# EntityOfCode/eoc-tfhe

Hardware: AMD Instinct MI355X
Metric: gate bootstraps/sec (HomNAND) (higher is better)
Workload: dtype f64

## Files before the change

eoc_tfhe_amd/csrc/blind_rotate_pair.inc:

```
    extern __shared__ __attribute__((aligned(16))) unsigned char smem[];
    d2 *s_tw = reinterpret_cast<d2 *>(smem);
    d2 *s_twist = s_tw + kTwEntries;
    d2 *s_scr_all = s_twist + kNH;

    const int tid = threadIdx.x, lane = tid & 63;
    const int h = __builtin_amdgcn_readfirstlane(tid >> 6);
    d2 *scr = s_scr_all + h * kScr;
    d2 *scr_partner = s_scr_all + (h ^ 1) * kScr;
    int32_t *ext = reinterpret_cast<int32_t *>(scr);

    const uint32_t job = blockIdx.x;
    typedef const __attribute__((address_space(4))) uint32_t *cu32p;
    unsigned long long bara_addr = (unsigned long long)(uintptr_t)(A.bara + (size_t)job * A.bara_stride);

    load_tables(s_tw, s_twist, g_tw, g_twist, tid, 128);
    if (A.prep && A.step_begin == 0) {
        const uint32_t gjob = A.job0 + job, g = gjob / A.ks_S;
        prepare_row(A.inline_desc ? A.desc0 : A.ks_descs[g], gjob - g * A.ks_S, A.n, A.bara + (size_t)job * A.bara_stride, tid, 128);
        if constexpr (SABAR) eoc_row_stores_to_l2();
        __syncthreads();
        if constexpr (SABAR) eoc_scalar_cache_acquire();
    }
    asm volatile("" : "+s"(bara_addr));
    const cu32p bara32 = (cu32p)bara_addr;
    uint16_t *s_abar = reinterpret_cast<uint16_t *>(s_scr_all + 2 * kScr);
    if constexpr (!SABAR) {
        const uint32_t *bara_v = reinterpret_cast<const uint32_t *>(A.bara + (size_t)job * A.bara_stride);
        for (int m = tid; m < (A.n + 2) / 2; m += 128) reinterpret_cast<uint32_t *>(s_abar)[m] = bara_v[m];
        __syncthreads();
    }
    auto load_abar = [&](int idx) __attribute__((always_inline)) {
        if constexpr (SABAR) return (int)((bara32[idx >> 1] >> ((idx & 1) * 16)) & 0xffffu);
        else return (int)s_abar[idx];
    };

    uint32_t racc[16];
    {
        const int barb = load_abar(A.n);
        const int rot = (2 * kN - barb) & (2 * kN - 1);
        const int32_t *st = A.acc_state + ((size_t)job * 2 + h) * kN;
        const int32_t *tvj = TV ? tv + (size_t)((A.job0 + job) / tv_rows) * kN : nullptr;
#pragma unroll
        for (int r = 0; r < 16; r++) {
            int j = lane + 64 * (r & 7) + (r >> 3) * kNH;
            int idx = (j - rot) & (2 * kN - 1);
            int32_t v;
            if constexpr (TV) {
                const uint32_t c = (uint32_t)tvj[idx & (kN - 1)];
                v = (int32_t)((idx & kN) ? 0u - c : c);
            } else {
                v = (idx & kN) ? -A.mu : A.mu;
            }
            v = h ? v : 0;
            if (A.step_begin > 0) v = st[j];
            racc[r] = (uint32_t)v;
        }
    }
    __syncthreads();

    const int Bgbit = BGBIT > 0 ? BGBIT : A.Bgbit;
    const uint32_t Bg = 1u << Bgbit, maskBg = Bg - 1, halfBg = Bg >> 1;
    uint32_t offset = 0;
#pragma unroll
    for (int p = 1; p <= L; p++) offset += halfBg << (32 - p * Bgbit);
    constexpr int KPL = 2 * L;
    const __amdgpu_buffer_rsrc_t bk_rsrc =
        __builtin_amdgcn_make_buffer_rsrc(const_cast<double *>(A.bkfft), 0, (int)((size_t)A.n * KPL * 2 * kNH * 16), 0x00020000);
    const double bias1 = 4503599627370496.0 + (double)halfBg, bias2 = 4503599627370496.0 + (double)Bg;

#ifdef EOC_STAMPS
    unsigned long long st_acc[16] = {0, 0, 0, 0, 0, 0, 0, 0, 0, 0, 0, 0, 0, 0, 0, 0};
    unsigned long long st_prev = __builtin_amdgcn_s_memtime();
    st_acc[12] = st_prev;
    st_acc[14] = __builtin_amdgcn_s_getreg((4) | (0 << 6) | (31 << 11));
    st_acc[13] = __builtin_amdgcn_s_getreg((20) | (0 << 6) | (31 << 11));
#endif
    const int prio_slot = __builtin_amdgcn_s_getreg((4) | (0 << 6) | (3 << 11));
    constexpr bool kResT2 = L == 2;
    d2 res_t2[4];
    if constexpr (kResT2) tw_load(res_t2, s_tw + kTwF2 + lane, 64);
    constexpr bool kResT1 = L == 2;
    d2 res_t1[4];
    if constexpr (kResT1) tw_load(res_t1, s_tw + kTwI1 + (lane & 7), 8);
    int abar_next = load_abar(A.step_begin);
    for (int i = A.step_begin; i < A.step_end; i++) {
        EOC_STAMP(15);
        if (A.prio_duty >= 0) {
            const bool first_part = (i & 15) < A.prio_duty;
            if (first_part == ((prio_slot & 1) != 0))
                __builtin_amdgcn_s_setprio(1);
            else
                __builtin_amdgcn_s_setprio(0);
        } else if (A.prio_duty <= -2) {
            const unsigned long long now = __builtin_amdgcn_s_memtime();
            if ((int)((now >> (-A.prio_duty)) & 1) == (prio_slot & 1))
                __builtin_amdgcn_s_setprio(1);
            else
                __builtin_amdgcn_s_setprio(0);
        }
        const int abar = __builtin_amdgcn_readfirstlane(abar_next);
        abar_next = load_abar(i + 1);
        auto load_row = [&](int p, int c, d2 (&b)[8]) __attribute__((always_inline)) {
            const uint32_t row_off = (uint32_t)((((size_t)i * KPL + h * L) * 2 + (size_t)(p - 1) * 2 + c) * kNH * 16);
#pragma unroll
            for (int r = 0; r < 8; r++)
                b[r] = __builtin_bit_cast(d2, __builtin_amdgcn_raw_buffer_load_b128(bk_rsrc, lane * 16, (int)(row_off + r * 1024), 0));
        };
        d2 ra[8], rb[8];
        uint32_t dlo[8], dhi[8];
        {
            const int s = abar & 63;
            const int src = ((lane - s) & 63) << 2;
            uint32_t t[16], d[16];
#pragma unroll
            for (int r = 0; r < 16; r++) t[r] = (uint32_t)__builtin_amdgcn_ds_bpermute(src, (int)racc[r]);
            const bool borrow = lane < s;
#define EOC_RQ(q) case q: rot_digits<q>(t, racc, borrow, offset, d); break;
            switch (abar >> 6) {
                EOC_RQ(0) EOC_RQ(1) EOC_RQ(2) EOC_RQ(3) EOC_RQ(4) EOC_RQ(5) EOC_RQ(6) EOC_RQ(7)
                EOC_RQ(8) EOC_RQ(9) EOC_RQ(10) EOC_RQ(11) EOC_RQ(12) EOC_RQ(13) EOC_RQ(14) EOC_RQ(15)
                EOC_RQ(16) EOC_RQ(17) EOC_RQ(18) EOC_RQ(19) EOC_RQ(20) EOC_RQ(21) EOC_RQ(22) EOC_RQ(23)
                EOC_RQ(24) EOC_RQ(25) EOC_RQ(26) EOC_RQ(27) EOC_RQ(28) EOC_RQ(29) EOC_RQ(30)
                default: rot_digits<31>(t, racc, borrow, offset, d); break;
            }
#undef EOC_RQ
#pragma unroll
            for (int r = 0; r < 8; r++) {
                dlo[r] = d[r];
                dhi[r] = d[8 + r];
            }
        }
        EOC_STAMP(0);
        auto make_x0 = [&](int p, d2 (&x)[8]) __attribute__((always_inline)) {
            const int shift = 32 - p * Bgbit;
#pragma unroll
            for (int r = 0; r < 4; r++) {
                const uint32_t ua = (dlo[r] >> shift) & maskBg, ub = (dhi[r] >> shift) & maskBg;
                const uint32_t up = (dlo[r + 4] >> shift) & maskBg, uq = (dhi[r + 4] >> shift) & maskBg;
                const double a = __hiloint2double(0x43300000, (int)ua) - bias1;
                const double b = __hiloint2double(0x43300000, (int)ub) - bias1;
                const double dm = __hiloint2double(0x43300000, (int)(up - uq + Bg)) - bias2;
                const double dp = __hiloint2double(0x43300000, (int)(up + uq)) - bias2;
                fwd_stage0(x[r], x[r + 4], a, b, dm, dp);
            }
            fwd_pass0_tail(x);
        };
        auto mac = [&](bool first, const d2 (&x)[8], const d2 (&b)[8], d2 (&acc_)[8]) __attribute__((always_inline)) {
#pragma unroll
            for (int r = 0; r < 8; r++) {
                if (first) {
                    acc_[r].x = EOC_FMA(-x[r].y, b[r].y, x[r].x * b[r].x);
                    acc_[r].y = EOC_FMA(x[r].y, b[r].x, x[r].x * b[r].y);
                } else {
                    acc_[r].x = EOC_FMA(-x[r].y, b[r].y, EOC_FMA(x[r].x, b[r].x, acc_[r].x));
                    acc_[r].y = EOC_FMA(x[r].y, b[r].x, EOC_FMA(x[r].x, b[r].y, acc_[r].y));
                }
            }
        };
        d2 xs[L][8], S[8];
#pragma unroll
        for (int p0 = 0; p0 + 1 < L; p0 += 2) {
            load_row(p0 + 1, 1 - h, ra);
            load_row(p0 + 2, 1 - h, rb);
            make_x0(p0 + 1, xs[p0]);
            EOC_STAMP(1);
            fft_fwd_rest_x2(xs[p0], xs[p0 + 1], [&]() __attribute__((always_inline)) { make_x0(p0 + 2, xs[p0 + 1]); },
                            s_tw, scr, lane, kResT2 ? &res_t2 : nullptr);
            EOC_STAMP(2);
            mac(p0 == 0, xs[p0], ra, S);
            mac(false, xs[p0 + 1], rb, S);
            EOC_STAMP(3);
        }
        if constexpr ((L & 1) != 0) {
            load_row(L, 1 - h, ra);
            make_x0(L, xs[L - 1]);
            EOC_STAMP(1);
            fft_fwd_rest(xs[L - 1], s_tw, scr, lane);
            EOC_STAMP(2);
            mac(L == 1, xs[L - 1], ra, S);
            EOC_STAMP(3);
        }
        load_row(1, h, ra);
        if constexpr (L >= 2) load_row(2, h, rb);
#pragma unroll
        for (int r = 0; r < 8; r++) scr[r * 64 + lane] = S[r];
        EOC_STAMP(4);
        __syncthreads();
        EOC_STAMP(5);
#pragma unroll
        for (int r = 0; r < 8; r++) S[r] = scr_partner[r * 64 + lane];
        mac(false, xs[0], ra, S);
        if constexpr (L >= 3) load_row(3, h, ra);
        if constexpr (L >= 2) mac(false, xs[1], rb, S);
        if constexpr (L >= 4) load_row(4, h, rb);
        if constexpr (L >= 3) mac(false, xs[2], ra, S);
        if constexpr (L >= 4) mac(false, xs[3], rb, S);
        EOC_STAMP(6);
        __syncthreads();
        EOC_STAMP(7);
        d2 ut[8];
        fft_inv_wave(S, ut, s_tw, s_twist, scr, lane, kResT1 ? &res_t1 : nullptr);
        EOC_STAMP(8);
#pragma unroll
        for (int r = 0; r < 8; r++) {
            d2 y = cmulc(S[r], ut[r]);
            racc[r] += wrap_trunc(y.x);
            racc[8 + r] += wrap_trunc(y.y);
        }
        wave_lds_fence();
        EOC_STAMP(9);
    }
    if (A.step_end >= A.n) {
#pragma unroll
        for (int r = 0; r < 16; r++) {
            const int j = lane + 64 * r;
            ext[j] = (int32_t)racc[r];
            ext[j + kN] = (int32_t)(0u - racc[r]);
        }
        wave_lds_fence();
    }
#ifdef EOC_STAMPS
    st_acc[11] = __builtin_amdgcn_s_memtime();
    if (A.stamps && lane == 0)
        for (int k = 0; k < 16; k++) A.stamps[((size_t)blockIdx.x * 2 + h) * 16 + k] = st_acc[k];
#endif

    const int lane_e = (int)__builtin_amdgcn_mbcnt_hi(~0u, __builtin_amdgcn_mbcnt_lo(~0u, 0u));
    if (A.step_end < A.n) {
        int32_t *st = A.acc_state + ((size_t)job * 2 + h) * kN;
#pragma unroll
        for (int r = 0; r < 16; r++) st[lane_e + 64 * (r & 7) + (r >> 3) * kNH] = (int32_t)racc[r];
        return;
    }
    if (MANY && !A.ks_descs) {
        const uint32_t gjob = A.job0 + job, g = gjob / tv_rows, si = gjob - g * tv_rows;
        int32_t *u0 = A.u - (size_t)A.job0 * (kN + 1) + ((size_t)g * n_tables * tv_rows + si) * (kN + 1);
        const size_t slot_stride = (size_t)tv_rows * (kN + 1);
        if (h == 0) {
            for (uint32_t jt = 0; jt < n_tables; jt++) {
                int32_t *u = u0 + jt * slot_stride;
#pragma unroll
                for (int r = 0; r < 16; r++) {
                    const int j = lane_e + 64 * r;
                    u[j] = ext[(2 * kN + (int)jt - j) & (2 * kN - 1)];
                }
            }
        } else if ((uint32_t)lane_e < n_tables) {
            u0[lane_e * slot_stride + kN] = ext[lane_e];
        }
    } else if (A.ks_descs) {
        const uint32_t gjob = A.job0 + job;
        if (h == 0) {
#pragma unroll
            for (int r = 0; r < 16; r++) {
// ... 22 lines not shown
```

eoc_tfhe_amd/csrc/engine.hip:

```cpp
#include "kernels.hip.h"
#include "canon_twiddles.h"
#include "common.h"
#include "../../include/eoc_tfhe_gpu.h"

#include <algorithm>
#include <cstdio>
#include <cstdlib>
#include <cstring>
#include <mutex>
#include <new>
#include <vector>

using namespace eoc;

#define HIP_TRY(expr)                                                                       \
    do {                                                                                    \
        hipError_t _e = (expr);                                                             \
        if (_e != hipSuccess) {                                                             \
            eoc_set_error("%s failed: %s (%s:%d)", #expr, hipGetErrorString(_e), __FILE__, \
                          __LINE__);                                                        \
            return EOC_ERR_HIP;                                                             \
        }                                                                                   \
    } while (0)

struct eoc_engine {
    int device = 0;
    eoc_params p{};
    int kpl = 0;
    size_t n1p = 0;
    d2 *d_tw = nullptr, *d_twist = nullptr;
    double *d_bkfft = nullptr;
    int32_t *d_ksk = nullptr;
    bool own_keys = false;
    const double *bkfft = nullptr;
    const int32_t *ksk = nullptr;
    void *d_ksl = nullptr;
    bool ksl_ready = false;
    struct Workspace {
        uint16_t *d_bara = nullptr;
        int32_t *d_u = nullptr;
        uint32_t *d_ubar = nullptr;
        int32_t *d_acc_state = nullptr;
        size_t ws_jobs = 0;
        GateDesc *d_descs = nullptr, *h_descs = nullptr;
        size_t ws_descs = 0, desc_pos = 0;
        hipEvent_t ring_ev = nullptr;
        bool ring_ev_set = false;
        bool ring_pushed_since_mark = false;
        GateDesc *d_persist = nullptr, *h_persist = nullptr;
        size_t persist_cap = 0, persist_pos = 0;
        int32_t *d_mixed = nullptr;
        uint32_t *h_perm = nullptr;
        hipEvent_t perm_ev = nullptr;
        size_t ws_mixed = 0;
    } ws;
    unsigned long long *d_stamps = nullptr;
    int num_cus = 256;
    int prio_duty_override = INT32_MIN;
    int prio_multi = -1;
    int br_slice = 0;
    bool no_fold = false;
    bool scalar_abar = false;
    bool no_pool = false;
    int br_parts = 0;
    int br_wide = -1;
    int bara_stride = 0;
    bool ks_waves_ok = true;
    int ks_mfma = -1;
    uint64_t stats[3] = {0, 0, 0};
    uint64_t ws_grows = 0;
    uint64_t br_launches = 0;
    uint64_t br_wide_launches = 0;
    uint64_t ks_mfma_launches = 0;
    bool profiling = false;
    struct Span { hipEvent_t a, b; int kind; };
    std::vector<Span> spans;
    double kernel_ms[3] = {0, 0, 0};
    uint64_t kernel_launches[3] = {0, 0, 0};
    std::mutex mu;
};

enum { KIND_PREPARE = 0, KIND_BLIND_ROTATE = 1, KIND_KEYSWITCH = 2 };

struct SpanGuard {
    eoc_engine *e;
    hipStream_t st;
    hipEvent_t a = nullptr, b = nullptr;
    int kind;
    SpanGuard(eoc_engine *e_, hipStream_t st_, int kind_) : e(e_), st(st_), kind(kind_)
    {
        if (!e->profiling) return;
        if (hipEventCreate(&a) != hipSuccess || hipEventCreate(&b) != hipSuccess) {
            a = b = nullptr;
            return;
        }
        hipEventRecord(a, st);
    }
    ~SpanGuard()
    {
        if (!a) return;
        hipEventRecord(b, st);
        e->spans.push_back({a, b, kind});
    }
};

static int valid_params(const eoc_params *p)
{
    if (!p) return 0;
    if (p->n < 1 || p->n > 1023) return 0;
    if (p->l < 1 || p->l > 4 || p->Bgbit < 1 || p->l * p->Bgbit > 32) return 0;
    if (((int64_t)p->l << p->Bgbit) > 8192) return 0;
    if (p->ks_t < 1 || p->ks_basebit < 1 || p->ks_basebit > 4 || p->ks_t * p->ks_basebit > 31) return 0;
    return 1;
}

extern "C" size_t eoc_bkfft_bytes(const eoc_params *p) { return (size_t)p->n * 2 * p->l * 2 * kNH * 16; }
extern "C" size_t eoc_ksk_row_stride(const eoc_params *p) { return ((size_t)p->n + 1 + 255) / 256 * 256; }
extern "C" size_t eoc_ksk_dev_bytes(const eoc_params *p)
{
    return (size_t)kN * p->ks_t * (((size_t)1 << p->ks_basebit) - 1) * eoc_ksk_row_stride(p) * 4;
// ... 53 lines not shown
        put(4 * lane, kTwI0 + 2 * 64 + lane);
        put(4 * (lane + 64), kTwI0 + 3 * 64 + lane);
    }
    for (int j = 0; j < kNH; j++) {
        twist[2 * j] = EOC_E2048[j][0];
        twist[2 * j + 1] = EOC_E2048[j][1];
    }
    HIP_TRY(hipMalloc(&e->d_tw, tw.size() * 8));
    HIP_TRY(hipMalloc(&e->d_twist, twist.size() * 8));
    HIP_TRY(hipMemcpy(e->d_tw, tw.data(), tw.size() * 8, hipMemcpyHostToDevice));
    HIP_TRY(hipMemcpy(e->d_twist, twist.data(), twist.size() * 8, hipMemcpyHostToDevice));
    HIP_TRY(hipDeviceSynchronize());
    return EOC_OK;
}

extern "C" int eoc_engine_create(int device, const eoc_params *p, eoc_engine **out)
{
    if (!out || !valid_params(p)) {
        eoc_set_error("eoc_engine_create: bad arguments (need 1 <= n <= 1023, 1 <= l <= 4, l * Bgbit <= 32, l * 2^Bgbit <= 8192 "
                      "-- the FP64 external product is not exact beyond that --, ks_t * ks_basebit <= 31, ks_basebit <= 4)");
        return EOC_ERR_ARG;
    }
    int cnt = eoc_device_count();
    if (cnt <= 0 || device < 0 || device >= cnt) {
        eoc_set_error("eoc_engine_create: no usable HIP device (count=%d, asked %d); the gate path has no CPU fallback",
                      cnt, device);
        return EOC_ERR_NO_DEVICE;
    }
    HIP_TRY(hipSetDevice(device));
    eoc_engine *e = new (std::nothrow) eoc_engine();
    if (!e) return EOC_ERR_ALLOC;
    e->device = device;
    e->p = *p;
    e->kpl = 2 * p->l;
    e->n1p = eoc_ksk_row_stride(p);
    e->bara_stride = (p->n + 1 + 31) / 32 * 32;
    int rc = upload_tables(e);
    if (rc) {
        delete e;
        return rc;
    }
    {
        int cus = 0;
        if (hipDeviceGetAttribute(&cus, hipDeviceAttributeMultiprocessorCount, device) == hipSuccess && cus > 0) e->num_cus = cus;
        if (const char *s = getenv("EOC_TFHE_PRIO_DUTY")) e->prio_duty_override = atoi(s);
        if (const char *s = getenv("EOC_TFHE_PRIO_MULTI")) e->prio_multi = atoi(s);
        if (const char *s = getenv("EOC_TFHE_BR_SLICE")) e->br_slice = atoi(s);
        if (getenv("EOC_TFHE_NO_FOLD")) e->no_fold = true;
        if (getenv("EOC_TFHE_NO_POOL")) e->no_pool = true;
        if (const char *s = getenv("EOC_TFHE_SCALAR_ABAR")) e->scalar_abar = atoi(s) != 0;
        if (const char *s = getenv("EOC_TFHE_BR_PARTS")) e->br_parts = atoi(s);
        if (const char *s = getenv("EOC_TFHE_BR_WIDE")) e->br_wide = atoi(s);
        if (const char *s = getenv("EOC_TFHE_KS_MFMA")) e->ks_mfma = atoi(s) != 0;
    }
#define EOC_KS_ATTR(TT, NWV, IWV)                                                                              \
    if (hipFuncSetAttribute(reinterpret_cast<const void *>(&k_keyswitch_waves<TT, NWV, IWV>),                  \
                            hipFuncAttributeMaxDynamicSharedMemorySize, KS3Cfg<TT, NWV, IWV>::LDS_BYTES) != hipSuccess) \
        e->ks_waves_ok = false
    EOC_KS_ATTR(8, 8, 16);
    EOC_KS_ATTR(8, 8, 32);
    EOC_KS_ATTR(8, 4, 64);
    EOC_KS_ATTR(8, 8, 64);
#undef EOC_KS_ATTR
    if (!e->ks_waves_ok) (void)hipGetLastError();
    *out = e;
    return EOC_OK;
}

static void free_ws(eoc_engine::Workspace &W)
{
    hipFree(W.d_bara);
    hipFree(W.d_u);
    hipFree(W.d_ubar);
    hipFree(W.d_acc_state);
    hipFree(W.d_descs);
    hipFree(W.d_mixed);
    if (W.h_descs) hipHostFree(W.h_descs);
    if (W.h_perm) hipHostFree(W.h_perm);
    if (W.perm_ev) hipEventDestroy(W.perm_ev);
    if (W.ring_ev) hipEventDestroy(W.ring_ev);
    hipFree(W.d_persist);
    if (W.h_persist) hipHostFree(W.h_persist);
    W = eoc_engine::Workspace();
}

extern "C" void eoc_engine_destroy(eoc_engine *e)
{
    if (!e) return;
    hipSetDevice(e->device);
    hipDeviceSynchronize();
    hipFree(e->d_tw);
    hipFree(e->d_twist);
    if (e->own_keys) {
        hipFree(e->d_bkfft);
        hipFree(e->d_ksk);
    }
    hipFree(e->d_ksl);
    free_ws(e->ws);
    hipFree(e->d_stamps);
    delete e;
}

static bool stream_is_capturing(hipStream_t st)
{
    hipStreamCaptureStatus cap = hipStreamCaptureStatusNone;
    return st && hipStreamIsCapturing(st, &cap) == hipSuccess && cap == hipStreamCaptureStatusActive;
// ... 280 lines not shown
        even(0, njobs_total, br_slice > 0 ? (uint32_t)br_slice : njobs_total, force_wide);
    else if (force_wide)
        even(0, njobs_total, resident_wide, true);
    else if (!can_wide || njobs_total <= resident_pair)
        even(0, njobs_total, resident_pair, false);
    else {
        const uint32_t full = njobs_total / resident_wide * resident_wide, rem = njobs_total - full;
        if (full) even(0, full, resident_wide, true);
        if (rem) even(full, rem, rem <= resident_pair ? resident_pair : resident_wide, rem > resident_pair);
    }
    return plan;
}

static BRArgs blind_rotate_args(const eoc_engine *e, const WS &W, const BRWork &w, const BRSeg &sg, int part, int parts)
{
    BRArgs a{};
    a.bkfft = e->bkfft;
    a.bara = W.d_bara + (size_t)sg.off * e->bara_stride;
    a.u = W.d_u + (size_t)sg.off * (kN + 1);
    a.njobs = sg.njobs;
    a.n = e->p.n;
    a.Bgbit = e->p.Bgbit;
    a.bara_stride = e->bara_stride;
    a.mu = (int32_t)(1u << 29);
    a.stamps = e->d_stamps;
    a.ks_descs = w.fold != BRWork::NONE ? w.descs : nullptr;
    a.prep = w.fold == BRWork::KS_AND_PREP;
    a.inline_desc = w.inline_desc != nullptr;
    if (w.inline_desc) {
        a.desc0 = *w.inline_desc;
        a.ks_descs = reinterpret_cast<const GateDesc *>(W.d_descs);
    }
    a.ubar = W.d_ubar;
    a.ks_S = w.fold != BRWork::NONE ? w.S : 1;
    a.ks_prec_offset = 1u << (32 - (1 + e->p.ks_basebit * e->p.ks_t));
    a.job0 = sg.off;
    a.step_begin = (int)((long long)e->p.n * part / parts);
    a.step_end = (int)((long long)e->p.n * (part + 1) / parts);
    a.acc_state = W.d_acc_state;
    const uint32_t resident = (sg.wide ? 8u : 4u) * (uint32_t)e->num_cus;
    a.prio_duty = (e->prio_duty_override != INT32_MIN) ? e->prio_duty_override
                  : (sg.njobs <= resident ? kPrioDuty : e->prio_multi);
    return a;
}

template <int L, int BGBIT> static const void *br_pair_kernel(BRWork::Seed seed, bool sabar)
{
    switch (seed) {
    case BRWork::GATE: return sabar ? (const void *)&k_blind_rotate<L, BGBIT, true> : (const void *)&k_blind_rotate<L, BGBIT, false>;
    case BRWork::TV: return sabar ? (const void *)&k_blind_rotate_tv<L, BGBIT, true> : (const void *)&k_blind_rotate_tv<L, BGBIT, false>;
    default: return sabar ? (const void *)&k_lut_many<L, BGBIT, true> : (const void *)&k_lut_many<L, BGBIT, false>;
    }
}
template <int BGBIT> static const void *br_wide_kernel(BRWork::Seed seed, bool sabar)
{
    switch (seed) {
    case BRWork::GATE: return sabar ? (const void *)&k_blind_rotate_wide<BGBIT, true> : (const void *)&k_blind_rotate_wide<BGBIT, false>;
    case BRWork::TV: return sabar ? (const void *)&k_blind_rotate_wide_tv<BGBIT, true> : (const void *)&k_blind_rotate_wide_tv<BGBIT, false>;
    default: return sabar ? (const void *)&k_lut_many_wide<BGBIT, true> : (const void *)&k_lut_many_wide<BGBIT, false>;
    }
}
struct BRKernel { const void *fn; dim3 grid, block; unsigned lds; };
static BRKernel blind_rotate_kernel(bool wide, int l, int Bgbit, bool sabar, BRWork::Seed seed, uint32_t njobs)
{
    if (wide) {
        const void *fn = Bgbit == 10 ? br_wide_kernel<10>(seed, sabar) : br_wide_kernel<0>(seed, sabar);
        return {fn, dim3((njobs + kBRWideJobsPerWG - 1) / kBRWideJobsPerWG), dim3(64 * kBRWideJobsPerWG), kBRWideLds};
    }
    const void *fn = nullptr;
    if (l == 2 && Bgbit == 10) fn = br_pair_kernel<2, 10>(seed, sabar);
    else if (l == 3 && Bgbit == 7) fn = br_pair_kernel<3, 7>(seed, sabar);
    else if (l == 1) fn = br_pair_kernel<1, 0>(seed, sabar);
    else if (l == 2) fn = br_pair_kernel<2, 0>(seed, sabar);
    else if (l == 3) fn = br_pair_kernel<3, 0>(seed, sabar);
    else if (l == 4) fn = br_pair_kernel<4, 0>(seed, sabar);
    return {fn, dim3(njobs), dim3(128), kBRLds};
}

static int launch_blind_rotate(eoc_engine *e, WS &W, const BRWork &w, hipStream_t st)
{
    const bool folds = w.fold != BRWork::NONE;
    if ((w.seed != BRWork::GATE && !w.tv) || (w.seed == BRWork::MANY && (folds || w.n_tables == 0)) ||
        (folds && !w.inline_desc && (!w.descs || !w.S)) || (w.inline_desc && (w.fold != BRWork::KS_AND_PREP || !w.S))) {
        eoc_set_error("internal: blind rotation of family %d with fold %d: a table family needs its test polynomials, the "
                      "many-LUT kernel has no fold, a fold needs descriptors and their row count", (int)w.seed, (int)w.fold);
        return EOC_ERR_STATE;
    }
    SpanGuard span(e, st, KIND_BLIND_ROTATE);
    const BRPlan plan = plan_blind_rotate(w.njobs, e->num_cus, e->p.l, e->kpl, e->p.n, e->br_slice, e->br_parts, e->br_wide);
    for (const BRSeg &sg : plan.segs) {
        const BRKernel k = blind_rotate_kernel(sg.wide, e->p.l, e->p.Bgbit, e->scalar_abar, w.seed, sg.njobs);
        if (!k.fn) return EOC_ERR_ARG;
        for (int part = 0; part < plan.parts; part++) {
            BRArgs a = blind_rotate_args(e, W, w, sg, part, plan.parts);
            void *args[] = {&a, (void *)&e->d_tw, (void *)&e->d_twist, (void *)&w.tv, (void *)&w.tv_rows, (void *)&w.n_tables};
            HIP_TRY(hipLaunchKernel(k.fn, k.grid, k.block, args, k.lds, st));
            e->br_launches++;
            e->br_wide_launches += sg.wide;
        }
    }
    return EOC_OK;
}

constexpr uint32_t kKsMfmaMinS = 1;
static int launch_keyswitch(eoc_engine *e, WS &W, const GateDesc *d_descs, uint32_t ngates, uint32_t S, hipStream_t st,
                            bool init_done, const GateDesc *inline_desc)
{
    KSArgs a;
    a.inline_desc = inline_desc != nullptr;
    if (inline_desc) a.desc0 = *inline_desc;
    else a.desc0 = GateDesc{0, 0, nullptr, nullptr, nullptr, nullptr};
    a.ksk = e->ksk;
    a.u = W.d_u;
    a.ubar = W.d_ubar;
    a.n = e->p.n;
    a.n1p = (int)e->n1p;
    a.t = e->p.ks_t;
    a.basebit = e->p.ks_basebit;
    a.S = S;
    a.mu = (int32_t)(1u << 29);
    SpanGuard span(e, st, KIND_KEYSWITCH);
    if (!init_done) {
        hipLaunchKernelGGL(k_ks_init, dim3(S, ngates), dim3(256), 0, st, d_descs, a);
        HIP_TRY(hipGetLastError());
    }
    const uint32_t ntiles = (S + KS_GT - 1) / KS_GT;
    const int ncb = (int)(e->n1p / 64);
    const int bb = e->p.ks_basebit, t = e->p.ks_t;
#define EOC_KS_LAUNCH(TT, NWV, IWV)                                                                     \
    do {                                                                                                  \
        auto kfn = k_keyswitch_waves<TT, NWV, IWV>;                                                       \
        constexpr int lds = KS3Cfg<TT, NWV, IWV>::LDS_BYTES;                                              \
        constexpr int ns = KS3Cfg<TT, NWV, IWV>::NS;                                                      \
        hipLaunchKernelGGL(kfn, dim3(ntiles * (unsigned)ncb * ns, ngates), dim3(64 * NWV), lds, st, d_descs, a); \
    } while (0)
    const bool fast = bb == 2 && t == 8 && e->ks_waves_ok;
    const bool mfma = bb == 2 && t == 8 && e->ksl_ready && (e->ks_mfma == 1 || (e->ks_mfma < 0 && S >= kKsMfmaMinS));
    if (mfma) {
        ks_mfma_launch(ks_mfma_plan(S, (int)e->n1p), ngates, d_descs, a, e->d_ksl, st);
        e->ks_mfma_launches++;
    }
    else if (fast && ncb == 4) EOC_KS_LAUNCH(8, 8, 16);
    else if (fast && ncb == 8) EOC_KS_LAUNCH(8, 8, 32);
    else if (fast && ncb == 12) EOC_KS_LAUNCH(8, 4, 64);
// ... 647 lines not shown
```

eoc_tfhe_amd/csrc/kernels.hip.h:

```cpp
#pragma once
#include <hip/hip_runtime.h>
#include <stdint.h>
#include <type_traits>

namespace eoc {

typedef double d2 __attribute__((ext_vector_type(2)));

constexpr int kN = 1024;
constexpr int kNH = 512;
constexpr int kScr = 568;
constexpr int kTwF1 = 0;
constexpr int kTwF2 = 32;
constexpr int kTwI1 = 32 + 256;
constexpr int kTwI0 = 32 + 256 + 32;
constexpr int kTwEntries = 32 + 256 + 32 + 256;

#define EOC_FMA(a, b, c) __builtin_fma((a), (b), (c))

#define EOC_SQRT_HALF 0x1.6a09e667f3bcdp-1
#define EOC_E128_RE 0x1.d906bcf328d46p-1
#define EOC_E128_IM 0x1.87de2a6aea963p-2
#define EOC_E64_RE 0x1.f6297cff75cb0p-1
#define EOC_E64_IM 0x1.8f8b83c69a60bp-3
// ... 97 lines not shown
    ct_w(x[0], x[2], t[1]);
    ct_w(x[1], x[3], t[1]);
    ct_iw(x[4], x[6], t[1]);
    ct_iw(x[5], x[7], t[1]);
    ct_w(x[0], x[1], t[2]);
    ct_iw(x[2], x[3], t[2]);
    ct_w(x[4], x[5], t[3]);
    ct_iw(x[6], x[7], t[3]);
}
__device__ __forceinline__ void t01_write(const d2 (&x)[8], d2 *scr, int lane)
{
#pragma unroll
    for (int r = 0; r < 8; r++) scr[72 * r + lane] = x[r];
    wave_lds_fence();
}
__device__ __forceinline__ void t01_read(d2 (&x)[8], const d2 *scr, int lane)
{
    const int hi = lane >> 3, lo = lane & 7;
#pragma unroll
    for (int r = 0; r < 8; r++) x[r] = scr[72 * hi + 8 * r + lo];
    wave_lds_fence();
}
__device__ __forceinline__ void t12_write(const d2 (&x)[8], d2 *scr, int lane)
{
    const int hi = lane >> 3, lo = lane & 7;
#pragma unroll
    for (int r = 0; r < 8; r++) scr[f12(hi * 64 + r * 8 + lo)] = x[r];
    wave_lds_fence();
}
__device__ __forceinline__ void t12_read(d2 (&x)[8], const d2 *scr, int lane)
{
#pragma unroll
    for (int r = 0; r < 8; r++) x[r] = scr[f12(lane * 8 + r)];
    wave_lds_fence();
}

__device__ __forceinline__ void fft_fwd_rest(d2 (&x)[8], const d2 *tw, d2 *scr, int lane)
{
    d2 t1[4], t2[4];
    tw_load(t1, tw + kTwF1 + (lane >> 3), 8);
    t01_write(x, scr, lane);
    t01_read(x, scr, lane);
    fwd_pass12(x, t1);
    t12_write(x, scr, lane);
    tw_load(t2, tw + kTwF2 + lane, 64);
    t12_read(x, scr, lane);
    fwd_pass12(x, t2);
}
#define EOC_SB() __builtin_amdgcn_sched_barrier(0)
#define EOC_SGB(mask, n) __builtin_amdgcn_sched_group_barrier((mask), (n), 0)
#define EOC_M_VALU 0x002
#define EOC_M_DSR 0x100
#define EOC_M_DSW 0x200
template <class MakeB>
__device__ __forceinline__ void fft_fwd_rest_x2(d2 (&xa)[8], d2 (&xb)[8], MakeB make_b, const d2 *tw, d2 *scr, int lane,
                                                const d2 (*T2)[4] = nullptr)
{
    d2 t1[4], t2[4];
    EOC_SB();
    tw_load(t1, tw + kTwF1 + (lane >> 3), 8);
    wave_lds_fence();
    t01_write(xa, scr, lane);
    make_b();
    t01_read(xa, scr, lane);
    EOC_SGB(EOC_M_DSR, 4);
#pragma unroll
    for (int k = 0; k < 8; k++) {
        EOC_SGB(EOC_M_DSW, 1);
        EOC_SGB(EOC_M_VALU, 10);
    }
    EOC_SGB(EOC_M_VALU, 64);
    EOC_SGB(EOC_M_DSR, 8);
    EOC_SB();
    t01_write(xb, scr, lane);
    t01_read(xb, scr, lane);
    if (T2) {
#pragma unroll
        for (int k = 0; k < 4; k++) t2[k] = (*T2)[k];
    } else {
        tw_load(t2, tw + kTwF2 + lane, 64);
    }
    wave_lds_fence();
    fwd_pass12(xa, t1);
#pragma unroll
    for (int k = 0; k < 8; k++) {
        EOC_SGB(EOC_M_DSW, 1);
        EOC_SGB(EOC_M_VALU, 4);
    }
    if (T2) EOC_SGB(EOC_M_DSR, 8);
    else EOC_SGB(EOC_M_DSR, 12);
    EOC_SGB(EOC_M_VALU, 40);
    EOC_SB();
    t12_write(xa, scr, lane);
    t12_read(xa, scr, lane);
    fwd_pass12(xb, t1);
#pragma unroll
    for (int k = 0; k < 8; k++) {
        EOC_SGB(EOC_M_DSW, 1);
        EOC_SGB(EOC_M_VALU, 4);
    }
    EOC_SGB(EOC_M_DSR, 8);
    EOC_SGB(EOC_M_VALU, 40);
    EOC_SB();
    t12_write(xb, scr, lane);
    t12_read(xb, scr, lane);
    fwd_pass12(xa, t2);
#pragma unroll
    for (int k = 0; k < 8; k++) {
        EOC_SGB(EOC_M_DSW, 1);
        EOC_SGB(EOC_M_VALU, 4);
    }
    EOC_SGB(EOC_M_DSR, 8);
    EOC_SGB(EOC_M_VALU, 40);
    EOC_SB();
    fwd_pass12(xb, t2);
}

__device__ __forceinline__ void inv_pass2(d2 (&x)[8])
{
    const d2 wc = {EOC_SQRT_HALF, EOC_SQRT_HALF};
    ct_1(x[0], x[1]);
    ct_1(x[2], x[3]);
    ct_1(x[4], x[5]);
    ct_1(x[6], x[7]);
    ct_1(x[0], x[2]);
    ct_ic(x[1], x[3]);
    ct_1(x[4], x[6]);
    ct_ic(x[5], x[7]);
    ct_1(x[0], x[4]);
    ct_wc(x[1], x[5], wc);
    ct_ic(x[2], x[6]);
    ct_iwc(x[3], x[7], wc);
}
__device__ __forceinline__ void inv_pass10(d2 (&x)[8], const d2 (&t)[4])
{
    ct_wc(x[0], x[1], t[0]);
    ct_wc(x[2], x[3], t[0]);
    ct_wc(x[4], x[5], t[0]);
    ct_wc(x[6], x[7], t[0]);
    ct_wc(x[0], x[2], t[1]);
    ct_iwc(x[1], x[3], t[1]);
    ct_wc(x[4], x[6], t[1]);
    ct_iwc(x[5], x[7], t[1]);
    ct_wc(x[0], x[4], t[2]);
    ct_wc(x[1], x[5], t[3]);
    ct_iwc(x[2], x[6], t[2]);
    ct_iwc(x[3], x[7], t[3]);
}
__device__ __forceinline__ void t21_read(d2 (&x)[8], const d2 *scr, int lane)
{
    const int hi = lane >> 3, lo = lane & 7;
#pragma unroll
    for (int r = 0; r < 8; r++) x[r] = scr[f12(hi * 64 + r * 8 + lo)];
    wave_lds_fence();
}
__device__ __forceinline__ void t10_read(d2 (&x)[8], const d2 *scr, int lane)
{
#pragma unroll
    for (int r = 0; r < 8; r++) x[r] = scr[72 * r + lane];
    wave_lds_fence();
}
__device__ __forceinline__ void fft_inv_wave(d2 (&x)[8], d2 (&ut)[8], const d2 *tw, const d2 *s_twist, d2 *scr, int lane,
                                             const d2 (*T1)[4] = nullptr)
{
    d2 t1[4], t0[4];
    EOC_SB();
    if (T1) {
#pragma unroll
        for (int k = 0; k < 4; k++) t1[k] = (*T1)[k];
    } else {
        tw_load(t1, tw + kTwI1 + (lane & 7), 8);
    }
    inv_pass2(x);
    {
        constexpr int ord[8] = {0, 4, 1, 5, 2, 6, 3, 7};
#pragma unroll
        for (int q = 0; q < 8; q++) scr[f12(lane * 8 + ord[q])] = x[ord[q]];
        wave_lds_fence();
    }
    t21_read(x, scr, lane);
    EOC_SGB(EOC_M_VALU, 32);
    EOC_SGB(EOC_M_VALU, 4);  EOC_SGB(EOC_M_DSW, 2);
    EOC_SGB(EOC_M_VALU, 6);  EOC_SGB(EOC_M_DSW, 2);
    EOC_SGB(EOC_M_VALU, 4);  EOC_SGB(EOC_M_DSW, 2);
    EOC_SGB(EOC_M_VALU, 6);  EOC_SGB(EOC_M_DSW, 2);
    EOC_SGB(EOC_M_DSR, 8);
    tw_load(t0, tw + kTwI0 + lane, 64);
#pragma unroll
    for (int r = 0; r < 8; r++) ut[r] = s_twist[lane + 64 * r];
    wave_lds_fence();
    EOC_SB();
    inv_pass10(x, t1);
    {
        constexpr int ord[8] = {0, 4, 1, 5, 2, 6, 3, 7};
        const int hi = lane >> 3, lo = lane & 7;
#pragma unroll
        for (int q = 0; q < 8; q++) scr[72 * hi + 8 * ord[q] + lo] = x[ord[q]];
        wave_lds_fence();
    }
    t10_read(x, scr, lane);
    EOC_SGB(EOC_M_VALU, 48);
#pragma unroll
    for (int k = 0; k < 4; k++) {
        EOC_SGB(EOC_M_VALU, 6);
        EOC_SGB(EOC_M_DSW, 2);
    }
    EOC_SGB(EOC_M_DSR, 8);
    EOC_SB();
    inv_pass10(x, t0);
}

__device__ __forceinline__ uint32_t wrap_trunc(double v)
{
    double m = __builtin_trunc(v) + 6755399441055744.0;
    return (uint32_t)__double2loint(m);
}

__device__ __forceinline__ void load_tables(d2 *s_tw, d2 *s_twist, const d2 *g_tw, const d2 *g_twist, int tid, int nthreads)
{
    for (int i = tid; i < kTwEntries; i += nthreads) s_tw[i] = g_tw[i];
    for (int i = tid; i < kNH; i += nthreads) s_twist[i] = g_twist[i];
}

__global__ __launch_bounds__(256) void k_fft_fwd_polys(const int32_t *__restrict__ polys,
                                                        double *__restrict__ specs, size_t count,
                                                        const d2 *__restrict__ g_tw,
                                                        const d2 *__restrict__ g_twist, double scale)
{
    __shared__ d2 s_tw[kTwEntries];
    __shared__ d2 s_scr[4][kScr];
    const int tid = threadIdx.x, lane = tid & 63, w = tid >> 6;
    for (int i = tid; i < kTwEntries; i += 256) s_tw[i] = g_tw[i];
    (void)g_twist;
    __syncthreads();
    size_t poly = (size_t)blockIdx.x * 4 + w;
    if (poly >= count) return;
    const int32_t *p = polys + poly * kN;
    d2 x[8];
#pragma unroll
    for (int r = 0; r < 4; r++) {
        int j = lane + 64 * r;
        double a = (double)p[j], b = (double)p[j + kNH], pp = (double)p[j + 256], q = (double)p[j + 256 + kNH];
// ... 173 lines not shown
        st_acc[k] += _t - st_prev;                                                        \
        st_prev = _t;                                                                     \
    } while (0)
#else
#define EOC_STAMP(k) do { } while (0)
#endif

struct BRArgs {
    const double *bkfft;
    uint16_t *bara;
    int32_t *u;
    uint32_t njobs;
    int n, Bgbit, bara_stride;
    int32_t mu;
    unsigned long long *stamps;
    int prio_duty;
    const GateDesc *ks_descs;
    GateDesc desc0;
    int inline_desc;
    int prep;
    uint32_t *ubar;
    uint32_t ks_S, ks_prec_offset, job0;
    int step_begin, step_end;
    int32_t *acc_state;
};

template <int Q>
__device__ __forceinline__ void rot_digits(const uint32_t (&t)[16], const uint32_t (&racc)[16], bool borrow, uint32_t offset,
                                           uint32_t (&d)[16])
{
#pragma unroll
    for (int r = 0; r < 16; r++) {
        const int k0 = (r - Q) & 31, k1 = (r - Q - 1) & 31;
        const uint32_t a0 = t[k0 & 15], a1 = t[k1 & 15];
        const uint32_t A = offset - racc[r];
        const bool n0 = k0 >= 16, n1 = k1 >= 16;
        if (n0 == n1) {
            const uint32_t w = borrow ? a1 : a0;
            d[r] = n0 ? A - w : A + w;
        } else {
            const uint32_t d0 = n0 ? A - a0 : A + a0, d1 = n1 ? A - a1 : A + a1;
            d[r] = borrow ? d1 : d0;
        }
    }
}
constexpr int kAbarLds = 2048;
constexpr int kBRLds = (kTwEntries + kNH + 2 * kScr) * 16 + kAbarLds;


template <int L, int BGBIT = 0, bool SABAR = false>
__global__ __launch_bounds__(128, 2) void k_blind_rotate(BRArgs A, const d2 *__restrict__ g_tw,
                                                         const d2 *__restrict__ g_twist)
{
    constexpr bool TV = false, MANY = false;
    const int32_t *const tv = nullptr;
    const uint32_t tv_rows = 1, n_tables = 1;
#include "blind_rotate_pair.inc"
}
template <int L, int BGBIT = 0, bool SABAR = false>
__global__ __launch_bounds__(128, 2) void k_blind_rotate_tv(BRArgs A, const d2 *__restrict__ g_tw,
                                                            const d2 *__restrict__ g_twist, const int32_t *__restrict__ tv,
                                                            uint32_t tv_rows)
{
    constexpr bool TV = true, MANY = false;
    const uint32_t n_tables = 1;
#include "blind_rotate_pair.inc"
}
template <int L, int BGBIT = 0, bool SABAR = false>
__global__ __launch_bounds__(128, 2) void k_lut_many(BRArgs A, const d2 *__restrict__ g_tw, const d2 *__restrict__ g_twist,
                                                     const int32_t *__restrict__ tv, uint32_t tv_rows, uint32_t n_tables)
{
    constexpr bool TV = true, MANY = true;
#include "blind_rotate_pair.inc"
}

__device__ __forceinline__ void fft_inv_x2(d2 (&xa)[8], d2 (&xb)[8], d2 (&ut)[8], const d2 *tw, const d2 *s_twist, d2 *scr,
                                           int lane)
{
    d2 t1[4], t0[4];
    const int hi = lane >> 3, lo = lane & 7;
    EOC_SB();
    tw_load(t1, tw + kTwI1 + (lane & 7), 8);
    inv_pass2(xa);
    EOC_SB();
#pragma unroll
    for (int r = 0; r < 8; r++) scr[f12(lane * 8 + r)] = xa[r];
    wave_lds_fence();
    inv_pass2(xb);
    t21_read(xa, scr, lane);
#pragma unroll
    for (int k = 0; k < 8; k++) {
        EOC_SGB(EOC_M_DSW, 1);
        EOC_SGB(EOC_M_VALU, 5);
    }
    EOC_SGB(EOC_M_VALU, 16);
    EOC_SGB(EOC_M_DSR, 8);
    EOC_SB();
#pragma unroll
    for (int r = 0; r < 8; r++) scr[f12(lane * 8 + r)] = xb[r];
    wave_lds_fence();
    t21_read(xb, scr, lane);
    tw_load(t0, tw + kTwI0 + lane, 64);
    wave_lds_fence();
    inv_pass10(xa, t1);
#pragma unroll
    for (int k = 0; k < 8; k++) {
        EOC_SGB(EOC_M_DSW, 1);
        EOC_SGB(EOC_M_VALU, 4);
    }
    EOC_SGB(EOC_M_DSR, 12);
    EOC_SGB(EOC_M_VALU, 40);
    EOC_SB();
#pragma unroll
    for (int r = 0; r < 8; r++) scr[72 * hi + 8 * r + lo] = xa[r];
    wave_lds_fence();
    t10_read(xa, scr, lane);
    inv_pass10(xb, t1);
#pragma unroll
    for (int k = 0; k < 8; k++) {
        EOC_SGB(EOC_M_DSW, 1);
        EOC_SGB(EOC_M_VALU, 4);
    }
    EOC_SGB(EOC_M_DSR, 8);
    EOC_SGB(EOC_M_VALU, 40);
    EOC_SB();
// ... 442 lines not shown
```

Measured before the change: 303,200.

## Keep L=2 blind-rotate twiddles in registers and software-pipeline bootstrapping-key row loads

For L=2 the blind-rotate kernel now loads the forward and inverse twiddles and the twist factors from global memory into registers once, and skips copying the tables into LDS. It also restructures the per-step MAC into a row-granular pipeline: bootstrapping-key rows are issued a few rows ahead, starting inside the last forward-FFT pass, and are interleaved with the MACs and the partner-scratch reads. The goal is to cut LDS traffic for twiddles and hide global-load latency. The cost is much higher register pressure, which could cause spills or lower occupancy. The old LDS-table path stays available through an environment flag.

```diff
diff --git a/eoc_tfhe_amd/csrc/blind_rotate_pair.inc b/eoc_tfhe_amd/csrc/blind_rotate_pair.inc
--- a/eoc_tfhe_amd/csrc/blind_rotate_pair.inc
+++ b/eoc_tfhe_amd/csrc/blind_rotate_pair.inc
@@ -13,7 +13,8 @@
     typedef const __attribute__((address_space(4))) uint32_t *cu32p;
     unsigned long long bara_addr = (unsigned long long)(uintptr_t)(A.bara + (size_t)job * A.bara_stride);
 
-    load_tables(s_tw, s_twist, g_tw, g_twist, tid, 128);
+    constexpr bool kResAll = L == 2 && !TLDS;
+    if constexpr (!kResAll) load_tables(s_tw, s_twist, g_tw, g_twist, tid, 128);
     if (A.prep && A.step_begin == 0) {
         const uint32_t gjob = A.job0 + job, g = gjob / A.ks_S;
         prepare_row(A.inline_desc ? A.desc0 : A.ks_descs[g], gjob - g * A.ks_S, A.n, A.bara + (size_t)job * A.bara_stride, tid, 128);
@@ -78,10 +79,19 @@
     const int prio_slot = __builtin_amdgcn_s_getreg((4) | (0 << 6) | (3 << 11));
     constexpr bool kResT2 = L == 2;
     d2 res_t2[4];
-    if constexpr (kResT2) tw_load(res_t2, s_tw + kTwF2 + lane, 64);
+    if constexpr (kResAll) tw_load(res_t2, g_tw + kTwF2 + lane, 64);
+    else if constexpr (kResT2) tw_load(res_t2, s_tw + kTwF2 + lane, 64);
     constexpr bool kResT1 = L == 2;
     d2 res_t1[4];
-    if constexpr (kResT1) tw_load(res_t1, s_tw + kTwI1 + (lane & 7), 8);
+    if constexpr (kResAll) tw_load(res_t1, g_tw + kTwI1 + (lane & 7), 8);
+    else if constexpr (kResT1) tw_load(res_t1, s_tw + kTwI1 + (lane & 7), 8);
+    d2 res_f1[4], res_i0[4], ut[8];
+    if constexpr (kResAll) {
+        tw_load(res_f1, g_tw + kTwF1 + (lane >> 3), 8);
+        tw_load(res_i0, g_tw + kTwI0 + lane, 64);
+#pragma unroll
+        for (int r = 0; r < 8; r++) ut[r] = g_twist[lane + 64 * r];
+    }
     int abar_next = load_abar(A.step_begin);
     for (int i = A.step_begin; i < A.step_end; i++) {
         EOC_STAMP(15);
@@ -106,7 +116,6 @@
             for (int r = 0; r < 8; r++)
                 b[r] = __builtin_bit_cast(d2, __builtin_amdgcn_raw_buffer_load_b128(bk_rsrc, lane * 16, (int)(row_off + r * 1024), 0));
         };
-        d2 ra[8], rb[8];
         uint32_t dlo[8], dhi[8];
         {
             const int s = abar & 63;
@@ -158,48 +167,105 @@
             }
         };
         d2 xs[L][8], S[8];
-#pragma unroll
-        for (int p0 = 0; p0 + 1 < L; p0 += 2) {
-            load_row(p0 + 1, 1 - h, ra);
-            load_row(p0 + 2, 1 - h, rb);
-            make_x0(p0 + 1, xs[p0]);
+        if constexpr (kResAll) {
+            constexpr int kRowAhead = 3;
+            const uint32_t step_off = (uint32_t)((((size_t)i * KPL + h * L) * 2) * kNH * 16);
+            d2 q[16][2];
+            auto issue = [&](int b) __attribute__((always_inline)) {
+                const uint32_t off = step_off + (uint32_t)((b < 8 ? 1 - h : h) * kNH * 16 + (b & 7) * 1024);
+                q[b][0] = __builtin_bit_cast(d2, __builtin_amdgcn_raw_buffer_load_b128(bk_rsrc, lane * 16, (int)off, 0));
+                q[b][1] = __builtin_bit_cast(d2, __builtin_amdgcn_raw_buffer_load_b128(bk_rsrc, lane * 16, (int)(off + 2 * kNH * 16), 0));
+            };
+            auto mac1 = [](d2 x, d2 b, d2 a) __attribute__((always_inline)) {
+                d2 o;
+                o.x = EOC_FMA(-x.y, b.y, EOC_FMA(x.x, b.x, a.x));
+                o.y = EOC_FMA(x.y, b.x, EOC_FMA(x.x, b.y, a.y));
+                return o;
+            };
+            make_x0(1, xs[0]);
             EOC_STAMP(1);
-            fft_fwd_rest_x2(xs[p0], xs[p0 + 1], [&]() __attribute__((always_inline)) { make_x0(p0 + 2, xs[p0 + 1]); },
-                            s_tw, scr, lane, kResT2 ? &res_t2 : nullptr);
+            fft_fwd_rest_x2(xs[0], xs[1], [&]() __attribute__((always_inline)) { make_x0(2, xs[1]); }, s_tw, scr, lane, &res_t2,
+                            &res_f1, [&]() __attribute__((always_inline)) {
+#pragma unroll
+                                for (int b = 0; b < kRowAhead; b++) issue(b);
+                            });
             EOC_STAMP(2);
-            mac(p0 == 0, xs[p0], ra, S);
-            mac(false, xs[p0 + 1], rb, S);
-            EOC_STAMP(3);
-        }
-        if constexpr ((L & 1) != 0) {
-            load_row(L, 1 - h, ra);
-            make_x0(L, xs[L - 1]);
-            EOC_STAMP(1);
-            fft_fwd_rest(xs[L - 1], s_tw, scr, lane);
-            EOC_STAMP(2);
-            mac(L == 1, xs[L - 1], ra, S);
-            EOC_STAMP(3);
-        }
-        load_row(1, h, ra);
-        if constexpr (L >= 2) load_row(2, h, rb);
-#pragma unroll
-        for (int r = 0; r < 8; r++) scr[r * 64 + lane] = S[r];
-        EOC_STAMP(4);
-        __syncthreads();
-        EOC_STAMP(5);
-#pragma unroll
-        for (int r = 0; r < 8; r++) S[r] = scr_partner[r * 64 + lane];
-        mac(false, xs[0], ra, S);
-        if constexpr (L >= 3) load_row(3, h, ra);
-        if constexpr (L >= 2) mac(false, xs[1], rb, S);
-        if constexpr (L >= 4) load_row(4, h, rb);
-        if constexpr (L >= 3) mac(false, xs[2], ra, S);
-        if constexpr (L >= 4) mac(false, xs[3], rb, S);
-        EOC_STAMP(6);
-        __syncthreads();
-        EOC_STAMP(7);
-        d2 ut[8];
-        fft_inv_wave(S, ut, s_tw, s_twist, scr, lane, kResT1 ? &res_t1 : nullptr);
+            EOC_SB();
+#pragma unroll
+            for (int r = 0; r < 8; r++) {
+                d2 s;
+                s.x = EOC_FMA(-xs[0][r].y, q[r][0].y, xs[0][r].x * q[r][0].x);
+                s.y = EOC_FMA(xs[0][r].y, q[r][0].x, xs[0][r].x * q[r][0].y);
+                s = mac1(xs[1][r], q[r][1], s);
+                scr[r * 64 + lane] = s;
+                EOC_SB();
+                issue(r + kRowAhead);
+                EOC_SB();
+            }
+            EOC_STAMP(4);
+            __syncthreads();
+            EOC_STAMP(5);
+            constexpr int kChainAhead = 2;
+#pragma unroll
+            for (int r = 0; r < kChainAhead; r++) S[r] = scr_partner[r * 64 + lane];
+            EOC_SB();
+#pragma unroll
+            for (int r = 0; r < 8; r++) {
+                S[r] = mac1(xs[0][r], q[8 + r][0], S[r]);
+                S[r] = mac1(xs[1][r], q[8 + r][1], S[r]);
+                EOC_SB();
+                if (r + kChainAhead < 8) S[r + kChainAhead] = scr_partner[(r + kChainAhead) * 64 + lane];
+                if (8 + r + kRowAhead < 16) issue(8 + r + kRowAhead);
+                EOC_SB();
+            }
+            EOC_STAMP(6);
+            __syncthreads();
+            EOC_STAMP(7);
+            fft_inv_wave<true>(S, ut, s_tw, s_twist, scr, lane, &res_t1, &res_i0);
+        } else {
+            d2 ra[8], rb[8];
+#pragma unroll
+            for (int p0 = 0; p0 + 1 < L; p0 += 2) {
+                load_row(p0 + 1, 1 - h, ra);
+                load_row(p0 + 2, 1 - h, rb);
+                make_x0(p0 + 1, xs[p0]);
+                EOC_STAMP(1);
+                fft_fwd_rest_x2(xs[p0], xs[p0 + 1], [&]() __attribute__((always_inline)) { make_x0(p0 + 2, xs[p0 + 1]); },
+                                s_tw, scr, lane, kResT2 ? &res_t2 : nullptr);
+                EOC_STAMP(2);
+                mac(p0 == 0, xs[p0], ra, S);
+                mac(false, xs[p0 + 1], rb, S);
+                EOC_STAMP(3);
+            }
+            if constexpr ((L & 1) != 0) {
+                load_row(L, 1 - h, ra);
+                make_x0(L, xs[L - 1]);
+                EOC_STAMP(1);
+                fft_fwd_rest(xs[L - 1], s_tw, scr, lane);
+                EOC_STAMP(2);
+                mac(L == 1, xs[L - 1], ra, S);
+                EOC_STAMP(3);
+            }
+            load_row(1, h, ra);
+            if constexpr (L >= 2) load_row(2, h, rb);
+#pragma unroll
+            for (int r = 0; r < 8; r++) scr[r * 64 + lane] = S[r];
+            EOC_STAMP(4);
+            __syncthreads();
+            EOC_STAMP(5);
+#pragma unroll
+            for (int r = 0; r < 8; r++) S[r] = scr_partner[r * 64 + lane];
+            mac(false, xs[0], ra, S);
+            if constexpr (L >= 3) load_row(3, h, ra);
+            if constexpr (L >= 2) mac(false, xs[1], rb, S);
+            if constexpr (L >= 4) load_row(4, h, rb);
+            if constexpr (L >= 3) mac(false, xs[2], ra, S);
+            if constexpr (L >= 4) mac(false, xs[3], rb, S);
+            EOC_STAMP(6);
+            __syncthreads();
+            EOC_STAMP(7);
+            fft_inv_wave(S, ut, s_tw, s_twist, scr, lane, kResT1 ? &res_t1 : nullptr);
+        }
         EOC_STAMP(8);
 #pragma unroll
         for (int r = 0; r < 8; r++) {
diff --git a/eoc_tfhe_amd/csrc/engine.hip b/eoc_tfhe_amd/csrc/engine.hip
--- a/eoc_tfhe_amd/csrc/engine.hip
+++ b/eoc_tfhe_amd/csrc/engine.hip
@@ -66,6 +66,7 @@
     int br_wide = -1;
     int bara_stride = 0;
     bool ks_waves_ok = true;
+    bool br_tables_lds = false;
     int ks_mfma = -1;
     uint64_t stats[3] = {0, 0, 0};
     uint64_t ws_grows = 0;
@@ -225,6 +226,7 @@
         if (const char *s = getenv("EOC_TFHE_BR_PARTS")) e->br_parts = atoi(s);
         if (const char *s = getenv("EOC_TFHE_BR_WIDE")) e->br_wide = atoi(s);
         if (const char *s = getenv("EOC_TFHE_KS_MFMA")) e->ks_mfma = atoi(s) != 0;
+        if (const char *s = getenv("EOC_TFHE_BR_TABLES_LDS")) e->br_tables_lds = atoi(s) != 0;
     }
 #define EOC_KS_ATTR(TT, NWV, IWV)                                                                              \
     if (hipFuncSetAttribute(reinterpret_cast<const void *>(&k_keyswitch_waves<TT, NWV, IWV>),                  \
@@ -611,6 +613,14 @@
     default: return sabar ? (const void *)&k_lut_many<L, BGBIT, true> : (const void *)&k_lut_many<L, BGBIT, false>;
     }
 }
+template <int L, int BGBIT> static const void *br_pair_lds_kernel(BRWork::Seed seed, bool sabar)
+{
+    switch (seed) {
+    case BRWork::GATE: return sabar ? (const void *)&k_br_lds<L, BGBIT, true> : (const void *)&k_br_lds<L, BGBIT, false>;
+    case BRWork::TV: return sabar ? (const void *)&k_br_lds_tv<L, BGBIT, true> : (const void *)&k_br_lds_tv<L, BGBIT, false>;
+    default: return sabar ? (const void *)&k_br_lds_many<L, BGBIT, true> : (const void *)&k_br_lds_many<L, BGBIT, false>;
+    }
+}
 template <int BGBIT> static const void *br_wide_kernel(BRWork::Seed seed, bool sabar)
 {
     switch (seed) {
@@ -620,14 +630,15 @@
     }
 }
 struct BRKernel { const void *fn; dim3 grid, block; unsigned lds; };
-static BRKernel blind_rotate_kernel(bool wide, int l, int Bgbit, bool sabar, BRWork::Seed seed, uint32_t njobs)
+static BRKernel blind_rotate_kernel(bool wide, int l, int Bgbit, bool sabar, bool tables_lds, BRWork::Seed seed, uint32_t njobs)
 {
     if (wide) {
         const void *fn = Bgbit == 10 ? br_wide_kernel<10>(seed, sabar) : br_wide_kernel<0>(seed, sabar);
         return {fn, dim3((njobs + kBRWideJobsPerWG - 1) / kBRWideJobsPerWG), dim3(64 * kBRWideJobsPerWG), kBRWideLds};
     }
     const void *fn = nullptr;
-    if (l == 2 && Bgbit == 10) fn = br_pair_kernel<2, 10>(seed, sabar);
+    if (l == 2 && tables_lds) fn = Bgbit == 10 ? br_pair_lds_kernel<2, 10>(seed, sabar) : br_pair_lds_kernel<2, 0>(seed, sabar);
+    else if (l == 2 && Bgbit == 10) fn = br_pair_kernel<2, 10>(seed, sabar);
     else if (l == 3 && Bgbit == 7) fn = br_pair_kernel<3, 7>(seed, sabar);
     else if (l == 1) fn = br_pair_kernel<1, 0>(seed, sabar);
     else if (l == 2) fn = br_pair_kernel<2, 0>(seed, sabar);
@@ -648,7 +659,7 @@
     SpanGuard span(e, st, KIND_BLIND_ROTATE);
     const BRPlan plan = plan_blind_rotate(w.njobs, e->num_cus, e->p.l, e->kpl, e->p.n, e->br_slice, e->br_parts, e->br_wide);
     for (const BRSeg &sg : plan.segs) {
-        const BRKernel k = blind_rotate_kernel(sg.wide, e->p.l, e->p.Bgbit, e->scalar_abar, w.seed, sg.njobs);
+        const BRKernel k = blind_rotate_kernel(sg.wide, e->p.l, e->p.Bgbit, e->scalar_abar, e->br_tables_lds, w.seed, sg.njobs);
         if (!k.fn) return EOC_ERR_ARG;
         for (int part = 0; part < plan.parts; part++) {
             BRArgs a = blind_rotate_args(e, W, w, sg, part, plan.parts);
diff --git a/eoc_tfhe_amd/csrc/kernels.hip.h b/eoc_tfhe_amd/csrc/kernels.hip.h
--- a/eoc_tfhe_amd/csrc/kernels.hip.h
+++ b/eoc_tfhe_amd/csrc/kernels.hip.h
@@ -173,18 +173,27 @@
 #define EOC_M_VALU 0x002
 #define EOC_M_DSR 0x100
 #define EOC_M_DSW 0x200
-template <class MakeB>
+struct FwdNoHook {
+    __device__ __forceinline__ void operator()() const {}
+};
+template <class MakeB, class BeforeLast = FwdNoHook>
 __device__ __forceinline__ void fft_fwd_rest_x2(d2 (&xa)[8], d2 (&xb)[8], MakeB make_b, const d2 *tw, d2 *scr, int lane,
-                                                const d2 (*T2)[4] = nullptr)
+                                                const d2 (*T2)[4] = nullptr, const d2 (*T1)[4] = nullptr,
+                                                BeforeLast before_last = BeforeLast())
 {
     d2 t1[4], t2[4];
     EOC_SB();
-    tw_load(t1, tw + kTwF1 + (lane >> 3), 8);
+    if (T1) {
+#pragma unroll
+        for (int k = 0; k < 4; k++) t1[k] = (*T1)[k];
+    } else {
+        tw_load(t1, tw + kTwF1 + (lane >> 3), 8);
+    }
     wave_lds_fence();
     t01_write(xa, scr, lane);
     make_b();
     t01_read(xa, scr, lane);
-    EOC_SGB(EOC_M_DSR, 4);
+    if (!T1) EOC_SGB(EOC_M_DSR, 4);
 #pragma unroll
     for (int k = 0; k < 8; k++) {
         EOC_SGB(EOC_M_DSW, 1);
@@ -234,6 +243,10 @@
     EOC_SGB(EOC_M_DSR, 8);
     EOC_SGB(EOC_M_VALU, 40);
     EOC_SB();
+    if constexpr (!std::is_same<BeforeLast, FwdNoHook>::value) {
+        before_last();
+        EOC_SB();
+    }
     fwd_pass12(xb, t2);
 }
 
@@ -281,8 +294,9 @@
     for (int r = 0; r < 8; r++) x[r] = scr[72 * r + lane];
     wave_lds_fence();
 }
+template <bool RESIDENT = false>
 __device__ __forceinline__ void fft_inv_wave(d2 (&x)[8], d2 (&ut)[8], const d2 *tw, const d2 *s_twist, d2 *scr, int lane,
-                                             const d2 (*T1)[4] = nullptr)
+                                             const d2 (*T1)[4] = nullptr, const d2 (*T0)[4] = nullptr)
 {
     d2 t1[4], t0[4];
     EOC_SB();
@@ -306,9 +320,14 @@
     EOC_SGB(EOC_M_VALU, 4);  EOC_SGB(EOC_M_DSW, 2);
     EOC_SGB(EOC_M_VALU, 6);  EOC_SGB(EOC_M_DSW, 2);
     EOC_SGB(EOC_M_DSR, 8);
-    tw_load(t0, tw + kTwI0 + lane, 64);
-#pragma unroll
-    for (int r = 0; r < 8; r++) ut[r] = s_twist[lane + 64 * r];
+    if constexpr (RESIDENT) {
+#pragma unroll
+        for (int k = 0; k < 4; k++) t0[k] = (*T0)[k];
+    } else {
+        tw_load(t0, tw + kTwI0 + lane, 64);
+#pragma unroll
+        for (int r = 0; r < 8; r++) ut[r] = s_twist[lane + 64 * r];
+    }
     wave_lds_fence();
     EOC_SB();
     inv_pass10(x, t1);
@@ -588,7 +607,7 @@
 __global__ __launch_bounds__(128, 2) void k_blind_rotate(BRArgs A, const d2 *__restrict__ g_tw,
                                                          const d2 *__restrict__ g_twist)
 {
-    constexpr bool TV = false, MANY = false;
+    constexpr bool TV = false, MANY = false, TLDS = false;
     const int32_t *const tv = nullptr;
     const uint32_t tv_rows = 1, n_tables = 1;
 #include "blind_rotate_pair.inc"
@@ -598,7 +617,7 @@
                                                             const d2 *__restrict__ g_twist, const int32_t *__restrict__ tv,
                                                             uint32_t tv_rows)
 {
-    constexpr bool TV = true, MANY = false;
+    constexpr bool TV = true, MANY = false, TLDS = false;
     const uint32_t n_tables = 1;
 #include "blind_rotate_pair.inc"
 }
@@ -606,7 +625,31 @@
 __global__ __launch_bounds__(128, 2) void k_lut_many(BRArgs A, const d2 *__restrict__ g_tw, const d2 *__restrict__ g_twist,
                                                      const int32_t *__restrict__ tv, uint32_t tv_rows, uint32_t n_tables)
 {
-    constexpr bool TV = true, MANY = true;
+    constexpr bool TV = true, MANY = true, TLDS = false;
+#include "blind_rotate_pair.inc"
+}
+
+template <int L, int BGBIT = 0, bool SABAR = false>
+__global__ __launch_bounds__(128, 2) void k_br_lds(BRArgs A, const d2 *__restrict__ g_tw, const d2 *__restrict__ g_twist)
+{
+    constexpr bool TV = false, MANY = false, TLDS = true;
+    const int32_t *const tv = nullptr;
+    const uint32_t tv_rows = 1, n_tables = 1;
+#include "blind_rotate_pair.inc"
+}
+template <int L, int BGBIT = 0, bool SABAR = false>
+__global__ __launch_bounds__(128, 2) void k_br_lds_tv(BRArgs A, const d2 *__restrict__ g_tw, const d2 *__restrict__ g_twist,
+                                                      const int32_t *__restrict__ tv, uint32_t tv_rows)
+{
+    constexpr bool TV = true, MANY = false, TLDS = true;
+    const uint32_t n_tables = 1;
+#include "blind_rotate_pair.inc"
+}
+template <int L, int BGBIT = 0, bool SABAR = false>
+__global__ __launch_bounds__(128, 2) void k_br_lds_many(BRArgs A, const d2 *__restrict__ g_tw, const d2 *__restrict__ g_twist,
+                                                        const int32_t *__restrict__ tv, uint32_t tv_rows, uint32_t n_tables)
+{
+    constexpr bool TV = true, MANY = true, TLDS = true;
 #include "blind_rotate_pair.inc"
 }
 
```

After: 309,000, median of 6. +1.9%, better.
